# qcc4cp/qcc

Measured on AMD Instinct MI355X. Metric: gate-applies/sec (2^30-amplitude units), QFT, higher is better.
Workload: dtype f64; 1 GPU; 30-qubit QFT complex128, 465 gates/step (qc.qft order), basis-state input, state resident in HBM, 2^30 amplitudes per GPU [BASELINE config 2]; qubits=30, fusion=1

## Files before the change

### qcc_amd/csrc/planner.h

```cpp
#pragma once
#include <sched.h>
#include <stdint.h>

#include <algorithm>
#include <atomic>
#include <cassert>
#include <cmath>
#include <cstdio>
#include <cstdlib>
#include <cstring>
#include <exception>
#include <new>
#include <string>
#include <thread>
#include <vector>

#include "../../include/qcc_hip.h"

namespace qh {

struct GateRec {
  uint64_t ctl_mask;
  int tgt;
  double g[8];
  uint64_t neg_mask = 0;
  uint8_t ghost = 0, variant = 0;
  uint8_t force_dense = 0;
};

inline bool is_diag(const double g[8]) {
  return g[2] == 0.0 && g[3] == 0.0 && g[4] == 0.0 && g[5] == 0.0;
}
inline bool is_one(double re, double im) { return re == 1.0 && im == 0.0; }
inline bool plan_diag(const double g[8], int tgt) {
  return is_diag(g) && (tgt < 0 || !(g[0] == 0.0 && g[1] == 0.0));
}
inline bool plan_diag(const GateRec &r) { return !r.force_dense && plan_diag(r.g, r.tgt); }

constexpr int kLaneBits = 6;
constexpr int kLaneLow = 3;
constexpr int kLaneHi = 3;
constexpr int kMaxLaneHiBit = 27;
constexpr int kMaxRegBits = 6;
inline int max_reg_bits(int bw) { return bw == 128 ? 5 : 6; }
constexpr int kMaxWaveBits = 2;
constexpr int kMaxSweepOps = 1024;
constexpr int kMaxInsertBits = 12;
constexpr int kMaxSlabBits = 3;

enum : uint32_t { OP_DENSE_REG = 0, OP_DENSE_LANE = 1, OP_DIAG = 2,
                  OP_LSWAP = 3,
                  OP_WSWAP = 4 };
enum : uint32_t { OPF_DEFER_C = 1, OPF_USE_C = 2, OPF_REAL = 4,
                  OPF_BFLY = 8, OPF_BFLY_SHIFT = 4,
                  OPF_LANE_DPP = 128, OPF_SWAP_RI = 256,
                  OPF_GHOST = 1024,
                  OPF_ROT_P = 2048, OPF_ROT_M = 4096 };

inline bool env_flag(const char *name, bool dflt) {
  const char *e = getenv(name);
  return e ? atoi(e) != 0 : dflt;
}

inline int env_int(const char *name, int dflt) {
  const char *e = getenv(name);
  return e ? atoi(e) : dflt;
}

struct PlanSwitches {
  bool wave_pinned = false;
  int wave_bits = 1;
  bool split_lanes = true;
  int max_rb = kMaxRegBits;
  bool bfly = true, propagate_x = true, defer_diag = true, rot_fuse = true;
  int lane_valu = 1, seats = 1;
  bool search = true, search_wb2 = true;
  bool steps_pinned = false; uint64_t steps = 0;
  int streams = 0;
  int only_wb = -1, pick = -1;
  int tiles_wb = 0;
  std::vector<std::vector<int>> tiles;
  bool threads = true, log = false, dag = false, verbose = false;

  static PlanSwitches from_env() {
    PlanSwitches w;
    if (const char *e = getenv("QH_WAVE_BITS")) { w.wave_pinned = true; w.wave_bits = std::max(0, std::min(kMaxWaveBits, atoi(e))); }
    w.split_lanes = env_flag("QH_SPLIT_LANES", true);
    w.max_rb = std::max(2, std::min(kMaxRegBits, env_int("QH_SWEEP_RB", kMaxRegBits)));
    w.bfly = env_flag("QH_BFLY", true), w.propagate_x = env_flag("QH_PROPAGATE_X", true);
    w.defer_diag = env_flag("QH_DEFER_DIAG", true), w.rot_fuse = env_flag("QH_ROT_FUSE", true);
    w.lane_valu = env_int("QH_LANE_VALU", 1), w.seats = env_int("QH_SEATS", 1);
    w.search = env_flag("QH_PLAN_SEARCH", true), w.search_wb2 = env_flag("QH_PLAN_SEARCH_WB2", true);
    if (const char *e = getenv("QH_PLAN_SEARCH_STEPS")) { w.steps_pinned = true; w.steps = strtoull(e, nullptr, 10); }
    if (const char *e = getenv("QH_PLAN_SEARCH_STREAMS")) w.streams = std::max(1, std::min(8, atoi(e)));
// ... 248 lines not shown
      pending.swap(rest);
      ++*nsweeps;
    }
  }

  void canonical_records(const std::vector<GateRec> &pending, std::vector<PassRec> *rec0, int back[64], uint64_t *movable) {
    const uint64_t always = (1ull << lane_low_) - 1;
    int canon[64], ncanon = lane_low_;
    for (int b = 0; b < 64; ++b) canon[b] = b < lane_low_ ? b : -1;
    auto canon_mask = [&](uint64_t m) {
      uint64_t o = 0;
      for (uint64_t t = m; t; t &= t - 1) {
        const int b = __builtin_ctzll(t);
        if (canon[b] < 0) canon[b] = ncanon++;
        o |= 1ull << canon[b];
      }
      return o;
    };
    rec0->resize(pending.size());
    uint64_t dense_used = 0;
    for (size_t i = 0; i < pending.size(); ++i) {
      const GateRec &r = pending[i];
      const bool diag = plan_diag(r);
      const uint64_t tb = canon_mask((r.tgt >= 0) ? (1ull << r.tgt) : 0);
      const uint64_t cb = canon_mask((r.ctl_mask | r.neg_mask) & ((1ull << nloc_) - 1));
      (*rec0)[i] = PassRec{diag ? 0 : tb, cb | (diag ? tb : 0), 1, tb ? __builtin_ctzll(tb) : -1};
      if (!diag) dense_used |= tb;
    }
    for (int b = 0; b < 64; ++b) back[b] = -1;
    for (int b = 0; b < 64; ++b) if (canon[b] >= 0) back[canon[b]] = b;
    *movable = dense_used & ~always;
  }
  static void build_dag(const std::vector<PassRec> &rec0, std::vector<int> *node_bit, std::vector<std::vector<int>> *succ,
                        std::vector<std::vector<int>> *pred) {
    int last_dense[64];
    std::vector<int> need[64];
    for (int b = 0; b < 64; ++b) last_dense[b] = -1;
    for (const PassRec &r : rec0) {
      if (!r.dense_bits) {
        for (uint64_t t = r.diag_bits; t; t &= t - 1) {
          const int b = __builtin_ctzll(t);
          for (uint64_t u = r.diag_bits & ~(1ull << b); u; u &= u - 1)
            if (last_dense[__builtin_ctzll(u)] >= 0) need[b].push_back(last_dense[__builtin_ctzll(u)]);
        }
        continue;
      }
      const int v = (int)node_bit->size(), tb = r.tgt;
      node_bit->push_back(tb);
      succ->emplace_back();
      pred->emplace_back();
      std::vector<int> ps;
      if (last_dense[tb] >= 0) ps.push_back(last_dense[tb]);
      for (int u : need[tb]) ps.push_back(u);
      for (uint64_t t = r.diag_bits; t; t &= t - 1) if (last_dense[__builtin_ctzll(t)] >= 0) ps.push_back(last_dense[__builtin_ctzll(t)]);
      std::sort(ps.begin(), ps.end());
      ps.erase(std::unique(ps.begin(), ps.end()), ps.end());
      for (int u : ps) { (*succ)[u].push_back(v); (*pred)[v].push_back(u); }
      need[tb].clear();
      last_dense[tb] = v;
      for (uint64_t t = r.diag_bits; t; t &= t - 1) need[__builtin_ctzll(t)].push_back(v);
    }
  }
  std::string dag_json(const std::vector<GateRec> &queue) {
    std::vector<GateRec> pending;
    std::vector<uint64_t> alg;
    uint64_t noops = 0;
    prepare(queue, &pending, &alg, &noops);
    std::vector<PassRec> rec0;
    int back[64];
    uint64_t movable = 0;
    canonical_records(pending, &rec0, back, &movable);
    std::vector<int> node_bit;
    std::vector<std::vector<int>> succ, pred;
    build_dag(rec0, &node_bit, &succ, &pred);
    std::string o = "{\"line_bits\":" + std::to_string(lane_low_) + ",\"cap_per_wave_bits\":[" + std::to_string(lane_hi_ + rb_cap_) + "," +
                    std::to_string(lane_hi_ + rb_cap_ + 1) + "," + std::to_string(lane_hi_ + rb_cap_ + 2) + "],\"target_bit\":[";
    for (size_t g = 0; g < node_bit.size(); ++g) o += (g ? "," : "") + std::to_string(back[node_bit[g]]);
    o += "],\"edges\":[";
    bool first = true;
    for (size_t u = 0; u < succ.size(); ++u)
      for (int v : succ[u]) { o += (first ? "[" : ",[") + std::to_string(u) + "," + std::to_string(v) + "]"; first = false; }
    return o + "]}";
  }
  bool search_levels(const std::vector<GateRec> &queue, size_t K, uint64_t change_budget, uint64_t stream,
                     std::vector<std::vector<int>> *tiles_out, uint64_t *changes_used = nullptr) {
    if (changes_used) *changes_used = 0;
    if (K < 2 || K > 8) return false;
    std::vector<GateRec> pending;
    std::vector<uint64_t> alg;
    uint64_t noops = 0;
    prepare(queue, &pending, &alg, &noops);
    std::vector<PassRec> rec0;
    int back[64];
    uint64_t movable = 0;
    canonical_records(pending, &rec0, back, &movable);
    const uint64_t always = (1ull << lane_low_) - 1;
    const int cap = lane_hi_ + rb_cap_ + max_wave_;
    if ((size_t)popc(movable) > K * (size_t)cap) return false;
    std::vector<int> node_bit;
    std::vector<std::vector<int>> succ, pred;
    build_dag(rec0, &node_bit, &succ, &pred);
    const int ng = (int)node_bit.size();
    if (!ng) return false;
    std::vector<int> depth(ng, 0);
    int maxd = 0;
    for (int u = 0; u < ng; ++u) for (int v : succ[u]) { depth[v] = std::max(depth[v], depth[u] + 1); maxd = std::max(maxd, depth[v]); }
    std::vector<int> chain[64];
    for (int g = 0; g < ng; ++g) chain[node_bit[g]].push_back(g);
    std::vector<int8_t> L(ng);
    int occ[64][8], ntile[8];
    uint64_t changes = 0;
    auto set_level = [&](int g, int to) {
      const int q = node_bit[g], from = L[g];
      ++changes;
      if (!((always >> q) & 1)) {
        if (--occ[q][from] == 0) --ntile[from];
        if (occ[q][to]++ == 0) ++ntile[to];
      }
      L[g] = (int8_t)to;
    };
    auto init = [&]() {
      memset(occ, 0, sizeof occ);
      memset(ntile, 0, sizeof ntile);
      for (int g = 0; g < ng; ++g) {
        L[g] = (int8_t)std::min<int>((int)K - 1, depth[g] * (int)K / (maxd + 1));
        const int q = node_bit[g];
        if (!((always >> q) & 1) && occ[q][L[g]]++ == 0) ++ntile[L[g]];
      }
    };
    auto cost = [&](int *over) {
      long sq = 0;
      int o = 0;
      for (size_t s = 0; s < K; ++s) { sq += (long)ntile[s] * ntile[s]; if (ntile[s] > cap) o += ntile[s] - cap; }
      *over = o;
      return (long)o * 100000 + sq;
    };
    std::vector<int> stk;
    std::vector<std::pair<int, int8_t>> undo;
    auto move = [&](int g, bool down) {
      const int to = L[g] + (down ? -1 : 1);
      if (to < 0 || to >= (int)K) return false;
      stk.assign(1, g);
      undo.emplace_back(g, L[g]);
      set_level(g, to);
      while (!stk.empty()) {
        const int u = stk.back();
        stk.pop_back();
        for (int v : down ? pred[u] : succ[u])
          if (down ? L[v] > to : L[v] < to) { undo.emplace_back(v, L[v]); set_level(v, to); stk.push_back(v); }
      }
      return true;
    };
    auto revert = [&]() { for (size_t i = undo.size(); i-- > 0;) set_level(undo[i].first, undo[i].second); undo.clear(); };
    uint64_t rng = 0x9e3779b97f4a7c15ull * (2 * stream + 1);
    auto rnd = [&](uint32_t n) { rng ^= rng << 13; rng ^= rng >> 7; rng ^= rng << 17; return (uint32_t)((rng >> 11) % n); };
    constexpr long kRestart = 1500;
    constexpr int kTenure = 7;
    std::vector<long> tabu((size_t)ng * 2);
    std::vector<int> cands;
    bool found = false;
    for (long walk = 0; !found; ++walk) {
      init();
      std::fill(tabu.begin(), tabu.end(), -1);
      int over = 0, best_over = 0;
      long best_key = cost(&best_over);
      over = best_over;
      for (long it = 0; it < kRestart && over > 0; ++it) {
        if (++changes > change_budget) goto out;
        if (walk == 0 && it == 400 && best_over > 4) goto out;
        cands.clear();
        for (size_t s = 0; s < K; ++s) {
          if (ntile[s] <= cap) continue;
          for (uint64_t t = movable; t; t &= t - 1) {
            const int q = __builtin_ctzll(t);
            if (!occ[q][s]) continue;
            int first = -1, last = -1;
            for (int g : chain[q]) if (L[g] == (int8_t)s) { if (first < 0) first = g; last = g; }
            cands.push_back(first * 2);
            cands.push_back(last * 2 + 1);
          }
        }
        long bk = 1L << 60;
        int bm = -1, ties = 0;
        for (int m : cands) {
          undo.clear();
          if (!move(m >> 1, m & 1)) continue;
          int o = 0;
          const long k = cost(&o);
          revert();
          if (tabu[m] > it && !(o < best_over)) continue;
          if (k < bk) { bk = k; bm = m; ties = 1; }
          else if (k == bk && rnd((uint32_t)++ties) == 0) bm = m;
        }
        if (bm < 0) continue;
        undo.clear();
        move(bm >> 1, bm & 1);
        const long k = cost(&over);
        for (const auto &u : undo) tabu[(size_t)u.first * 2 + ((bm & 1) ? 0 : 1)] = it + kTenure + (long)rnd(kTenure);
        if (k < best_key) { best_key = k; best_over = over; }
      }
      found = over == 0;
    }
  out:
    if (changes_used) *changes_used = changes;
    if (!found) return false;
    tiles_out->clear();
    for (size_t s = 0; s < K; ++s) {
      std::vector<int> b;
      for (uint64_t t = movable; t; t &= t - 1) if (occ[__builtin_ctzll(t)][s]) b.push_back(back[__builtin_ctzll(t)]);
      std::sort(b.begin(), b.end());
      tiles_out->push_back(b);
    }
    return true;
  }
  void set_tiles(const std::vector<std::vector<int>> &t) { tiles_ = t; }

  PlanResult plan(const std::vector<GateRec> &queue) {
    PlanResult out;
    std::vector<GateRec> pending;
    std::vector<uint64_t> alg;
    prepare(queue, &pending, &alg, &out.noop_gates);
    const uint64_t lm = (1ull << nloc_) - 1;
    std::vector<int> first_tile;
    keep_line_bits_ = !tiles_.empty();
    while (!pending.empty()) {
      std::vector<GateRec> rest;
      std::vector<uint64_t> rest_alg;
      std::vector<uint32_t> rest_w;
      std::vector<int> forced;
      const std::vector<int> *fs = nullptr;
      if (out.sweeps.size() < tiles_.size()) {
        for (int b : tiles_[out.sweeps.size()])
          if (b >= lane_low_ && b < nloc_) forced.push_back(out.final_pos[b]);
        fs = &forced;
      }
      out.sweeps.push_back(build_sweep(pending, alg, &rest, &rest_alg, &rest_w, fs));
      if (out.sweeps.size() == 1) {
        const SweepPlan &f = out.sweeps[0];
        for (int k = 0; k < f.nlanehi(); ++k) first_tile.push_back(f.lanehi[k]);
        for (int k = 0; k < f.rb; ++k) first_tile.push_back(f.regpos[k]);
        for (int k = 0; k < f.nwave; ++k) first_tile.push_back(f.wavepos[k]);
      }
      if (out.sweeps.back().relayout) {
        std::vector<int> ahead;
        if (!rest.empty() && out.sweeps.size() < tiles_.size()) {
          for (int b : tiles_[out.sweeps.size()])
            if (b >= lane_low_ && b < nloc_) ahead.push_back(out.final_pos[b]);
        } else if (!rest.empty()) {
          select_tile_bits(rest, &ahead);
        } else if (out.sweeps.size() > 1) {
          for (int p : first_tile) ahead.push_back(out.final_pos[p]);
        }
        std::sort(ahead.begin(), ahead.end());
        finish_relayout(&out.sweeps.back(), ahead);
        if (unit_segments(out.sweeps.back(), nloc_, nullptr, nullptr) > kMaxUnitSegs)
          finish_relayout(&out.sweeps.back(), std::vector<int>());
      }
      const SweepPlan &done = out.sweeps.back();
      if (done.relayout) {
        auto map_mask = [&](uint64_t m) {
          uint64_t o = m >> nloc_ << nloc_;
          for (uint64_t t = m & lm; t; t &= t - 1) o |= 1ull << done.dest_pos[__builtin_ctzll(t)];
          return o;
        };
        for (GateRec &r : rest) {
          r.ctl_mask = map_mask(r.ctl_mask);
          r.neg_mask = map_mask(r.neg_mask);
          if (r.tgt >= 0 && r.tgt < nloc_) r.tgt = done.dest_pos[r.tgt];
        }
        for (int p = 0; p < nloc_; ++p) out.final_pos[p] = done.dest_pos[out.final_pos[p]];
        out.moved = true;
      }
      pending.swap(rest);
      alg.swap(rest_alg);
      weight_.swap(rest_w);
    }
    return out;
  }

 private:
  int nloc_;
  uint64_t shard_;
  uint64_t amp_bytes_;
  int rb_cap_;
  int lane_low_ = kLaneLow, lane_hi_ = kLaneHi;
  bool split_lanes_;
  bool relayout_;
  bool keep_ghosts_;
  bool butterflies_;
  static constexpr size_t dense_weight_ = 1;
  int max_wave_;
  bool propagate_x_;
  static constexpr bool store_swapped_ = true, lanes_by_count_ = true, lanes_high_ = true, bitfac_ = true, fold_sink_ = true;
  static constexpr int min_table_terms_ = 2;
  bool fold_pending_ = false;
  bool keep_line_bits_ = false;
  double fold_re_ = 1, fold_im_ = 0;
// ... 1076 lines not shown
        const int i = __builtin_ctz(g.reg_mask & ~(1u << best_j));
        for (int t = 0; t < no; ++t) if (others[t] == i) slot = t;
      }
      if (slot < 0) { kept.push_back(g); continue; }
      cmul_acc(&w[2 * slot], &w[2 * slot + 1], g.re, g.im);
      if ((int)k < base_abs) base--;
    }
    if (base < 0) {
      DGroup g{};
      g.reg_mask = 1u << best_j;
      g.re = 1; g.im = 0;
      kept.push_back(g);
      base = (int)kept.size() - 1;
    } else {
      base -= (int)first;
    }
    kept[base].flags |= DG_BITFAC;
    kept[base].tab_off[3] = (uint32_t)(sp->tables.size() / 2);
    for (double x : w) sp->tables.push_back(x);
    sp->groups.resize(first);
    for (const DGroup &g : kept) sp->groups.push_back(g);
  }
};

inline bool plan_has_far_tile(const PlanResult &pr) {
  for (const SweepPlan &sp : pr.sweeps) {
    int far = 0;
    for (int k = 0; k < sp.nlanehi(); ++k) far += sp.lanehi[k] >= 25;
    for (int k = 0; k < sp.rb; ++k) far += sp.regpos[k] >= 25;
    if (far >= 8) return true;
  }
  return false;
}

inline double sweep_op_energy_nj(const SweepPlan &sp) {
  const double nr = (double)(1u << sp.rb);
  double e = 0;
  for (const SweepOp &op : sp.ops) {
    const uint32_t f = op.flags;
    if (f & OPF_GHOST) continue;
    switch (op.kind) {
      case OP_DENSE_REG:
        if ((f & OPF_BFLY) && (f & (OPF_ROT_P | OPF_ROT_M))) e += 3 * nr * 1.58;
        else if (f & OPF_BFLY) e += 2 * nr * 1.5;
        else if (f & OPF_REAL) e += 5 * nr * 1.9;
        else e += (10 * nr + 10) * 1.95;
        break;
      case OP_DENSE_LANE:
        if ((f & OPF_LANE_DPP) && (f & OPF_BFLY)) e += (nr * (op.tb == 2 ? 10 : 6) + 14) * 1.0;
        else if (f & OPF_LANE_DPP) e += (nr * (op.tb == 2 ? 12 : 8) + 20) * 1.1;
        else if (f & OPF_BFLY) e += (2 * nr + 8) * 1.5 + 4 * nr * 1.0;
        else e += (((f & OPF_REAL) ? 4 : 10) * nr + 30) * 1.9 + 4 * nr * 1.0;
        break;
      case OP_LSWAP: e += (2 * nr + 8) * 1.2; break;
      case OP_WSWAP: e += 5 * 1.0 + 2 * nr * 1.0; break;
      case OP_DIAG: {
        bool c_touched = false, c_sign = false;
        for (uint32_t gi = 0; gi < op.n_groups; ++gi) {
          const DGroup &g = sp.groups[op.group_off + gi];
          const double slots = nr / (double)(1u << popc((uint64_t)g.reg_mask));
          const bool general = (g.flags & DG_LTAB) || g.ntab || g.n_oterms;
          const bool sign = g.re == -1.0 && g.im == 0.0 && !(g.flags & DG_LTAB) && !g.ntab;
          if (g.flags & DG_BITFAC) { e += (124 + ((g.lane_mask || general) ? 11 : 0)) * 1.95; continue; }
          if (sign) {
            if (!g.reg_mask) { e += 6 * 1.0; c_touched = c_sign = true; }
            else e += (4 + 2 * slots) * 1.0;
            continue;
          }
          double pro = 0;
          if (general) pro = 4 + 4 * g.ntab + 4 * g.n_oterms + ((g.flags & DG_LTAB) ? 4 : 7);
          else if (g.lane_mask) pro = 11;
          if (!g.reg_mask) { e += (pro + 4) * 1.9; c_touched = true; c_sign = false; }
          else e += 4 * slots * 1.95 + pro * 1.0;
        }
        if (c_touched && !(f & OPF_DEFER_C)) e += (c_sign ? (2 * nr + 1) : 4 * nr) * 1.95;
        break;
      }
      default: break;
    }
  }
  return e;
}

inline double plan_predicted_ms(const PlanResult &pr, int nloc, int bw) {
  double ms = 0;
  for (const SweepPlan &sp : pr.sweeps) {
    const double scale = (double)sp.swept_bytes / (2.0 * 16.0 * (double)(1ull << 30));
    const double e_ops_j = sweep_op_energy_nj(sp) * (double)sp.ntiles * 1e-9;
    const double floor_ms = (sp.nwave >= 2 ? 6.0 : 5.5) * scale;
    ms += std::max(floor_ms, 3.0 * scale + 0.99 * e_ops_j) + (sp.nwave >= 2 ? 0.3 * scale : 0.0);
  }
  (void)nloc; (void)bw;
  return ms;
}

inline unsigned usable_cpus() {
  unsigned n = std::thread::hardware_concurrency();
  cpu_set_t set;
  if (sched_getaffinity(0, sizeof set, &set) == 0) { const int c = CPU_COUNT(&set); if (c > 0 && (!n || (unsigned)c < n)) n = (unsigned)c; }
  for (const char *path : {"/sys/fs/cgroup/cpu.max", "/sys/fs/cgroup/cpu/cpu.cfs_quota_us"}) {
    FILE *f = fopen(path, "r");
    if (!f) continue;
    long long quota = -1, period = 100000;
    char word[32] = {0};
    if (fscanf(f, "%31s %lld", word, &period) >= 1 && strcmp(word, "max") != 0) quota = atoll(word);
    fclose(f);
    if (strstr(path, "cfs_quota")) {
      period = 100000;
      if (FILE *g = fopen("/sys/fs/cgroup/cpu/cpu.cfs_period_us", "r")) { if (fscanf(g, "%lld", &period) != 1) period = 100000; fclose(g); }
    }
    if (quota > 0 && period > 0) { const unsigned q = (unsigned)std::max<long long>(1, quota / period); if (!n || q < n) n = q; }
    break;
  }
  return n;
}

inline PlanResult plan_best(const std::vector<GateRec> &queue, const PlanRequest &rq) {
  const PlanSwitches &sw = rq.sw;
  const int nloc = rq.nloc, bw = rq.bw;
  const bool keep_ghosts = rq.keep_ghosts;
  if (sw.wave_pinned) return Planner(rq).plan(queue);
  if (!sw.tiles.empty()) {
    Planner forced(rq, sw.tiles_wb);
    forced.set_tiles(sw.tiles);
    return forced.plan(queue);
  }
  int best_wb = 1;
  size_t best_n = 0, n_of[kMaxWaveBits + 1] = {0, 0, 0};
  bool have = false, best_far = false, far_of[kMaxWaveBits + 1] = {false, false, false};
  const int only_wb = sw.only_wb;
  for (int wb : {1, 2, 0}) {
    if (only_wb >= 0 && wb != only_wb) continue;
    size_t n = 0;
    bool far = false;
    Planner(rq, wb).skeleton(queue, &n, &far);
    n_of[wb] = n;
    far_of[wb] = far;
    if (!have || (best_far && !far) || (best_far == far && n < best_n)) {
      best_wb = wb;
      best_n = n;
      best_far = far;
      have = true;
    }
    if (best_n <= 1 && !best_far) break;
  }
  Planner chosen(rq, best_wb);
  uint64_t dense_bits = 0;
  for (const GateRec &q : queue) if (q.tgt >= 0 && q.tgt < nloc && !plan_diag(q.g, q.tgt)) dense_bits |= 1ull << q.tgt;
  const int lane_low = bw == 128 ? 3 : 4;
  const int cap0 = (kLaneBits - lane_low) + std::min({sw.max_rb, max_reg_bits(bw), nloc - kLaneBits});
  if (best_n >= 3 && sw.search) {
    const double sweep_us = 2.0 * (double)(bw == 128 ? 16 : 8) * (double)(1ull << nloc) / 5.5e6;
    const uint64_t budget = sw.steps_pinned ? sw.steps : std::min<uint64_t>((uint64_t)(sweep_us * 640.0), 5000000);
    struct Task {
      int wb;
      size_t K;
      uint64_t stream, used = 0;
      bool ok = false, planned = false;
      double ms = 0;
      PlanResult pr;
      std::exception_ptr failed;
    };
    std::vector<Task> tasks;
    const size_t nmovable = (size_t)popc(dense_bits >> lane_low);
    std::vector<std::pair<int, size_t>> shapes;
    for (int wb : {1, 2, 0}) {
      if (budget < 5000) break;
      if (wb != best_wb && (wb == 0 || far_of[wb] || n_of[wb] == 0 || best_n < 4 || (wb == 2 && !sw.search_wb2))) continue;
      if (only_wb >= 0 && wb != only_wb) continue;
      const size_t cap = (size_t)(cap0 + wb), greedy = n_of[wb];
      const size_t kmin = std::max<size_t>({2, (nmovable + cap - 1) / cap, greedy > 3 ? greedy - 3 : 0});
      for (size_t K = kmin; K + 1 <= greedy && K <= best_n && K <= 8; ++K) shapes.emplace_back(wb, K);
    }
    int streams = 6;
    if (const unsigned hw = usable_cpus(); hw && !keep_ghosts && !shapes.empty())
      streams = std::max(1, std::min(6, (int)(hw / shapes.size())));
    if (sw.streams) streams = sw.streams;
    for (const auto &sh : shapes)
      for (int s = 0; s < streams; ++s) { tasks.emplace_back(); tasks.back().wb = sh.first; tasks.back().K = sh.second; tasks.back().stream = (uint64_t)(s + 1); }
    auto run = [&](Task &t) {
      const size_t i = (size_t)(&t - &tasks[0]);
      try {
        std::vector<std::vector<int>> tiles;
        t.ok = Planner(rq, t.wb).search_levels(queue, t.K, budget, t.stream, &tiles, &t.used);
        if (!t.ok) return;
        Planner forced(rq, t.wb);
        forced.set_tiles(tiles);
        t.pr = forced.plan(queue);
        t.planned = t.pr.sweeps.size() <= t.K && !plan_has_far_tile(t.pr);
      } catch (...) { t.failed = std::current_exception(); return; }
      if (t.planned) t.ms = keep_ghosts ? 1000.0 * (double)t.pr.sweeps.size() + 1e-3 * (double)(i + 1) : plan_predicted_ms(t.pr, nloc, bw);
    };
    std::atomic<size_t> next{0};
    auto drain = [&] { for (size_t i; (i = next++) < tasks.size(); ) run(tasks[i]); };
    std::vector<std::thread> pool;
    const size_t workers = sw.threads ? std::min<size_t>(tasks.size(), usable_cpus()) : 0;
    try { while (pool.size() < workers) pool.emplace_back(drain); } catch (...) {}
    PlanResult greedy_plan;
    std::exception_ptr greedy_failed;
    try { greedy_plan = chosen.plan(queue); } catch (...) { greedy_failed = std::current_exception(); next = tasks.size(); }
    drain();
    for (std::thread &x : pool) x.join();
    if (greedy_failed) std::rethrow_exception(greedy_failed);
    const Task *win = nullptr;
    double best_ms = keep_ghosts ? 1000.0 * (double)greedy_plan.sweeps.size() : plan_predicted_ms(greedy_plan, nloc, bw);
    for (const Task &t : tasks)
      if (t.planned && t.pr.sweeps.size() <= greedy_plan.sweeps.size() && t.ms < best_ms) { win = &t; best_ms = t.ms; }
    if (sw.pick >= 0) {
      if ((size_t)sw.pick < tasks.size() && tasks[sw.pick].planned) win = &tasks[sw.pick];
    }
    if (sw.log) {
      for (const Task &t : tasks)
        fprintf(stderr, "[qh plan search]   task %d: wave bits %d K=%zu stream %llu: %s after %llu label changes%s\n", (int)(&t - &tasks[0]), t.wb, t.K, (unsigned long long)t.stream,
                t.failed ? "FAILED (exception)" : t.ok ? "found" : "not found", (unsigned long long)t.used,
                t.planned ? (", " + std::to_string(t.pr.sweeps.size()) + " sweeps, predicted " + std::to_string(t.ms) + " ms").c_str() : "");
      fprintf(stderr, "[qh plan search] greedy: %d wave bit(s), %zu sweeps, predicted %.2f ms; chosen: %s (%zu tasks, budget %llu label changes each)\n", best_wb,
              greedy_plan.sweeps.size(), plan_predicted_ms(greedy_plan, nloc, bw),
              win ? (std::to_string(win->pr.sweeps.size()) + " sweeps with " + std::to_string(win->wb) + " wave bit(s), predicted " + std::to_string(win->ms) + " ms").c_str() : "greedy",
              tasks.size(), (unsigned long long)budget);
    }
    if (keep_ghosts)
      for (const Task &t : tasks) if (t.failed) std::rethrow_exception(t.failed);
    if (win) return win->pr;
    return greedy_plan;
  }
  return chosen.plan(queue);
}

template <class F> int guard_planning(std::string *err, F &&f) {
  try { f(); } catch (const std::bad_alloc &) { *err = "planning: out of host memory"; return QH_ERR_NOMEM; }
  catch (const std::exception &e) { *err = std::string("planning: ") + e.what(); return QH_ERR_ARG; }
  return QH_OK;
}

inline std::string plan_to_json(const std::vector<GateRec> &queue, const PlanRequest &rq) {
  if (rq.nloc < kLaneBits + 2) return "{\"sweeps\":[],\"note\":\"state too small for sweeps\"}";
  PlanResult pr = plan_best(queue, rq);
  std::string s = "{\"noop_gates\":" + std::to_string(pr.noop_gates);
  if (rq.sw.dag)
    s += ",\"dag\":" + Planner(rq, 1).dag_json(queue);
  s += ",\"sweeps\":[";
  char buf[384];
  for (size_t i = 0; i < pr.sweeps.size(); ++i) {
    const SweepPlan &sp = pr.sweeps[i];
    int nd = 0, ndiag = 0, nbf = 0;
    int nswap = 0, ndpp = 0;
    for (auto &o : sp.ops) {
      if (o.kind == OP_LSWAP || o.kind == OP_WSWAP) { nswap++; continue; }
      (o.kind == OP_DIAG ? ndiag : nd)++;
      if (o.flags & OPF_BFLY) nbf++;
      if (o.flags & OPF_LANE_DPP) ndpp++;
    }
    std::string rp = "[";
    for (int k = 0; k < sp.rb; ++k) rp += (k ? "," : "") + std::to_string(sp.regpos[k]);
    rp += "],\"lanehi\":[";
    for (int k = 0; k < sp.nlanehi(); ++k) rp += (k ? "," : "") + std::to_string(sp.lanehi[k]);
    rp += "],\"wavepos\":[";
    for (int k = 0; k < sp.nwave; ++k) rp += (k ? "," : "") + std::to_string(sp.wavepos[k]);
    rp += "]";
    rp += sp.relayout ? ",\"relayout\":1" : ",\"relayout\":0";
    snprintf(buf, sizeof buf,
             "%s{\"gates\":%llu,\"dense_ops\":%d,\"butterfly_ops\":%d,\"dpp_ops\":%d,\"lswap_ops\":%d,\"diag_ops\":%d,\"groups\":%zu,\"oterms\":%zu,\"table_entries\":%zu,"
             "\"regpos\":%s,\"fixed_ones\":%llu,\"ntiles\":%llu,\"alg_bytes\":%llu,\"swept_bytes\":%llu}",
             i ? "," : "", (unsigned long long)sp.gates, nd, nbf, ndpp, nswap, ndiag, sp.groups.size(), sp.oterms.size(),
             sp.tables.size() / 2, rp.c_str(), (unsigned long long)sp.fixed_ones, (unsigned long long)sp.ntiles,
             (unsigned long long)sp.alg_bytes, (unsigned long long)sp.swept_bytes);
    s += buf;
    if (rq.sw.verbose) {
      s.pop_back();
      s += ",\"ops\":[";
      for (size_t k = 0; k < sp.ops.size(); ++k) {
        const SweepOp &o = sp.ops[k];
        snprintf(buf, sizeof buf, "%s{\"kind\":%u,\"tb\":%u,\"flags\":%u,\"cm_reg\":%u,\"cm_thread\":%llu,\"groups\":[",
                 k ? "," : "", o.kind, o.tb, o.flags, o.cm_reg, (unsigned long long)o.cm_thread);
        s += buf;
        for (uint32_t gi = 0; o.kind == OP_DIAG && gi < o.n_groups; ++gi) {
          const DGroup &g = sp.groups[o.group_off + gi];
          snprintf(buf, sizeof buf, "%s[%u,%u,%u,%u,%u,%.17g,%.17g]", gi ? "," : "", g.lane_mask, g.reg_mask, g.flags, g.ntab, g.n_oterms, g.re, g.im);
          s += buf;
        }
        s += "]}";
      }
      s += "]}";
    }
  }
  s += "]}";
  return s;
}

}
```

Before: 27540 gate-applies/s.

## Run plan search in budgeted rounds with pruning and a DAG lower bound

The tabu level search becomes a resumable LevelSearch object, and plan_best runs it over several rounds with doubling budgets. After each round it drops tasks that cannot beat the incumbent plan, and it adds extra streams for promising shapes onto spare CPUs. A new DAG-span lower bound (min_tile_slots) raises the minimum sweep count K so hopeless shapes are never searched. The aim is to cut planning time and spend search effort where it can help, but pruning may drop a search that would have found a better plan, which changes the kernel schedule chosen.

```diff
diff --git a/qcc_amd/csrc/planner.h b/qcc_amd/csrc/planner.h
--- a/qcc_amd/csrc/planner.h
+++ b/qcc_amd/csrc/planner.h
@@ -10,6 +10,8 @@
 #include <cstdlib>
 #include <cstring>
 #include <exception>
+#include <functional>
+#include <memory>
 #include <new>
 #include <string>
 #include <thread>
@@ -424,10 +426,7 @@
       for (int v : succ[u]) { o += (first ? "[" : ",[") + std::to_string(u) + "," + std::to_string(v) + "]"; first = false; }
     return o + "]}";
   }
-  bool search_levels(const std::vector<GateRec> &queue, size_t K, uint64_t change_budget, uint64_t stream,
-                     std::vector<std::vector<int>> *tiles_out, uint64_t *changes_used = nullptr) {
-    if (changes_used) *changes_used = 0;
-    if (K < 2 || K > 8) return false;
+  size_t min_tile_slots(const std::vector<GateRec> &queue, int cap) {
     std::vector<GateRec> pending;
     std::vector<uint64_t> alg;
     uint64_t noops = 0;
@@ -436,125 +435,209 @@
     int back[64];
     uint64_t movable = 0;
     canonical_records(pending, &rec0, back, &movable);
-    const uint64_t always = (1ull << lane_low_) - 1;
-    const int cap = lane_hi_ + rb_cap_ + max_wave_;
-    if ((size_t)popc(movable) > K * (size_t)cap) return false;
     std::vector<int> node_bit;
     std::vector<std::vector<int>> succ, pred;
     build_dag(rec0, &node_bit, &succ, &pred);
-    const int ng = (int)node_bit.size();
-    if (!ng) return false;
-    std::vector<int> depth(ng, 0);
-    int maxd = 0;
-    for (int u = 0; u < ng; ++u) for (int v : succ[u]) { depth[v] = std::max(depth[v], depth[u] + 1); maxd = std::max(maxd, depth[v]); }
-    std::vector<int> chain[64];
-    for (int g = 0; g < ng; ++g) chain[node_bit[g]].push_back(g);
-    std::vector<int8_t> L(ng);
-    int occ[64][8], ntile[8];
-    uint64_t changes = 0;
-    auto set_level = [&](int g, int to) {
-      const int q = node_bit[g], from = L[g];
-      ++changes;
-      if (!((always >> q) & 1)) {
-        if (--occ[q][from] == 0) --ntile[from];
-        if (occ[q][to]++ == 0) ++ntile[to];
-      }
-      L[g] = (int8_t)to;
-    };
-    auto init = [&]() {
-      memset(occ, 0, sizeof occ);
-      memset(ntile, 0, sizeof ntile);
-      for (int g = 0; g < ng; ++g) {
-        L[g] = (int8_t)std::min<int>((int)K - 1, depth[g] * (int)K / (maxd + 1));
-        const int q = node_bit[g];
-        if (!((always >> q) & 1) && occ[q][L[g]]++ == 0) ++ntile[L[g]];
-      }
-    };
-    auto cost = [&](int *over) {
+    const size_t ng = node_bit.size(), nw = (ng + 63) / 64;
+    auto is_movable = [&](int g) { return (movable >> node_bit[g]) & 1; };
+    std::vector<uint64_t> below(ng * nw, 0), above(ng * nw, 0);
+    for (size_t u = ng; u-- > 0;) {
+      below[u * nw + u / 64] |= 1ull << (u % 64);
+      for (int v : succ[u]) for (size_t w = 0; w < nw; ++w) below[u * nw + w] |= below[(size_t)v * nw + w];
+    }
+    for (size_t v = 0; v < ng; ++v) {
+      above[v * nw + v / 64] |= 1ull << (v % 64);
+      for (int u : pred[v]) for (size_t w = 0; w < nw; ++w) above[v * nw + w] |= above[(size_t)u * nw + w];
+    }
+    size_t events = 0;
+    int last[64];
+    for (int b = 0; b < 64; ++b) last[b] = -1;
+    struct Pair { int q; std::vector<uint64_t> span; bool open; };
+    std::vector<Pair> pairs;
+    for (size_t g = 0; g < ng; ++g) {
+      if (!is_movable((int)g)) continue;
+      ++events;
+      const int q = node_bit[g], f = last[q];
+      last[q] = (int)g;
+      if (f < 0) continue;
+      Pair p{q, std::vector<uint64_t>(nw), true};
+      uint64_t targets = 0;
+      for (size_t w = 0; w < nw; ++w) {
+        p.span[w] = below[(size_t)f * nw + w] & above[g * nw + w];
+        for (uint64_t t = p.span[w]; t; t &= t - 1) targets |= 1ull << node_bit[w * 64 + __builtin_ctzll(t)];
+      }
+      if (popc(targets & movable) <= cap) pairs.push_back(std::move(p));
+    }
+    size_t merges = 0, left = pairs.size();
+    std::vector<size_t> in_spans(ng);
+    while (left) {
+      std::fill(in_spans.begin(), in_spans.end(), 0);
+      for (const Pair &p : pairs)
+        if (p.open) for (size_t w = 0; w < nw; ++w) for (uint64_t t = p.span[w]; t; t &= t - 1) ++in_spans[w * 64 + __builtin_ctzll(t)];
+      const size_t x = (size_t)(std::max_element(in_spans.begin(), in_spans.end()) - in_spans.begin());
+      size_t per_qubit[64] = {0};
+      for (Pair &p : pairs)
+        if (p.open && ((p.span[x / 64] >> (x % 64)) & 1)) { ++per_qubit[p.q]; p.open = false; --left; }
+      std::sort(per_qubit, per_qubit + 64, std::greater<size_t>());
+      for (int k = 0; k < cap && k < 64; ++k) merges += per_qubit[k];
+    }
+    return events - merges;
+  }
+
+  class LevelSearch {
+   public:
+    enum State { kRunning, kFound, kGaveUp };
+    LevelSearch(const PlanRequest &rq, int wave_bits, const std::vector<GateRec> &queue, size_t K, uint64_t stream)
+        : K_(K), rng_(0x9e3779b97f4a7c15ull * (2 * stream + 1)) {
+      if (K < 2 || K > 8) { state_ = kGaveUp; return; }
+      Planner pl(rq, wave_bits);
+      std::vector<GateRec> pending;
+      std::vector<uint64_t> alg;
+      uint64_t noops = 0;
+      pl.prepare(queue, &pending, &alg, &noops);
+      std::vector<PassRec> rec0;
+      pl.canonical_records(pending, &rec0, back_, &movable_);
+      always_ = (1ull << pl.lane_low_) - 1;
+      cap_ = pl.lane_hi_ + pl.rb_cap_ + pl.max_wave_;
+      if ((size_t)popc(movable_) > K * (size_t)cap_) { state_ = kGaveUp; return; }
+      build_dag(rec0, &node_bit_, &succ_, &pred_);
+      ng_ = (int)node_bit_.size();
+      if (!ng_) { state_ = kGaveUp; return; }
+      depth_.assign(ng_, 0);
+      for (int u = 0; u < ng_; ++u) for (int v : succ_[u]) { depth_[v] = std::max(depth_[v], depth_[u] + 1); maxd_ = std::max(maxd_, depth_[v]); }
+      for (int g = 0; g < ng_; ++g) chain_[node_bit_[g]].push_back(g);
+      L_.resize(ng_);
+      tabu_.resize((size_t)ng_ * 2);
+    }
+    State state() const { return state_; }
+    uint64_t changes() const { return changes_; }
+    int least_overflow() const { return least_over_; }
+
+    State run(uint64_t change_budget) {
+      constexpr long kRestart = 1500;
+      constexpr int kTenure = 7;
+      while (state_ == kRunning) {
+        if (!in_walk_) {
+          init();
+          std::fill(tabu_.begin(), tabu_.end(), -1);
+          best_key_ = cost(&best_over_);
+          over_ = best_over_;
+          least_over_ = std::min(least_over_, best_over_);
+          it_ = 0;
+          in_walk_ = true;
+        }
+        for (; it_ < kRestart && over_ > 0; ++it_) {
+          if (changes_ + 1 > change_budget) return state_;
+          ++changes_;
+          if (walk_ == 0 && it_ == 400 && best_over_ > kFarOverflow) return state_ = kGaveUp;
+          cands_.clear();
+          for (size_t s = 0; s < K_; ++s) {
+            if (ntile_[s] <= cap_) continue;
+            for (uint64_t t = movable_; t; t &= t - 1) {
+              const int q = __builtin_ctzll(t);
+              if (!occ_[q][s]) continue;
+              int first = -1, last = -1;
+              for (int g : chain_[q]) if (L_[g] == (int8_t)s) { if (first < 0) first = g; last = g; }
+              cands_.push_back(first * 2);
+              cands_.push_back(last * 2 + 1);
+            }
+          }
+          long bk = 1L << 60;
+          int bm = -1, ties = 0;
+          for (int m : cands_) {
+            undo_.clear();
+            if (!move(m >> 1, m & 1)) continue;
+            int o = 0;
+            const long k = cost(&o);
+            revert();
+            if (tabu_[m] > it_ && !(o < best_over_)) continue;
+            if (k < bk) { bk = k; bm = m; ties = 1; }
+            else if (k == bk && rnd((uint32_t)++ties) == 0) bm = m;
+          }
+          if (bm < 0) continue;
+          undo_.clear();
+          move(bm >> 1, bm & 1);
+          const long k = cost(&over_);
+          for (const auto &u : undo_) tabu_[(size_t)u.first * 2 + ((bm & 1) ? 0 : 1)] = it_ + kTenure + (long)rnd(kTenure);
+          if (k < best_key_) { best_key_ = k; best_over_ = over_; }
+          least_over_ = std::min(least_over_, over_);
+        }
+        in_walk_ = false;
+        ++walk_;
+        if (over_ == 0) state_ = kFound;
+      }
+      return state_;
+    }
+    std::vector<std::vector<int>> tiles() const {
+      std::vector<std::vector<int>> out;
+      for (size_t s = 0; s < K_; ++s) {
+        std::vector<int> b;
+        for (uint64_t t = movable_; t; t &= t - 1) if (occ_[__builtin_ctzll(t)][s]) b.push_back(back_[__builtin_ctzll(t)]);
+        std::sort(b.begin(), b.end());
+        out.push_back(b);
+      }
+      return out;
+    }
+    static constexpr int kFarOverflow = 4;
+
+   private:
+    void set_level(int g, int to) {
+      const int q = node_bit_[g], from = L_[g];
+      ++changes_;
+      if (!((always_ >> q) & 1)) {
+        if (--occ_[q][from] == 0) --ntile_[from];
+        if (occ_[q][to]++ == 0) ++ntile_[to];
+      }
+      L_[g] = (int8_t)to;
+    }
+    void init() {
+      memset(occ_, 0, sizeof occ_);
+      memset(ntile_, 0, sizeof ntile_);
+      for (int g = 0; g < ng_; ++g) {
+        L_[g] = (int8_t)std::min<int>((int)K_ - 1, depth_[g] * (int)K_ / (maxd_ + 1));
+        const int q = node_bit_[g];
+        if (!((always_ >> q) & 1) && occ_[q][L_[g]]++ == 0) ++ntile_[L_[g]];
+      }
+    }
+    long cost(int *over) const {
       long sq = 0;
       int o = 0;
-      for (size_t s = 0; s < K; ++s) { sq += (long)ntile[s] * ntile[s]; if (ntile[s] > cap) o += ntile[s] - cap; }
+      for (size_t s = 0; s < K_; ++s) { sq += (long)ntile_[s] * ntile_[s]; if (ntile_[s] > cap_) o += ntile_[s] - cap_; }
       *over = o;
       return (long)o * 100000 + sq;
-    };
-    std::vector<int> stk;
-    std::vector<std::pair<int, int8_t>> undo;
-    auto move = [&](int g, bool down) {
-      const int to = L[g] + (down ? -1 : 1);
-      if (to < 0 || to >= (int)K) return false;
-      stk.assign(1, g);
-      undo.emplace_back(g, L[g]);
+    }
+    bool move(int g, bool down) {
+      const int to = L_[g] + (down ? -1 : 1);
+      if (to < 0 || to >= (int)K_) return false;
+      stk_.assign(1, g);
+      undo_.emplace_back(g, L_[g]);
       set_level(g, to);
-      while (!stk.empty()) {
-        const int u = stk.back();
-        stk.pop_back();
-        for (int v : down ? pred[u] : succ[u])
-          if (down ? L[v] > to : L[v] < to) { undo.emplace_back(v, L[v]); set_level(v, to); stk.push_back(v); }
+      while (!stk_.empty()) {
+        const int u = stk_.back();
+        stk_.pop_back();
+        for (int v : down ? pred_[u] : succ_[u])
+          if (down ? L_[v] > to : L_[v] < to) { undo_.emplace_back(v, L_[v]); set_level(v, to); stk_.push_back(v); }
       }
       return true;
-    };
-    auto revert = [&]() { for (size_t i = undo.size(); i-- > 0;) set_level(undo[i].first, undo[i].second); undo.clear(); };
-    uint64_t rng = 0x9e3779b97f4a7c15ull * (2 * stream + 1);
-    auto rnd = [&](uint32_t n) { rng ^= rng << 13; rng ^= rng >> 7; rng ^= rng << 17; return (uint32_t)((rng >> 11) % n); };
-    constexpr long kRestart = 1500;
-    constexpr int kTenure = 7;
-    std::vector<long> tabu((size_t)ng * 2);
-    std::vector<int> cands;
-    bool found = false;
-    for (long walk = 0; !found; ++walk) {
-      init();
-      std::fill(tabu.begin(), tabu.end(), -1);
-      int over = 0, best_over = 0;
-      long best_key = cost(&best_over);
-      over = best_over;
-      for (long it = 0; it < kRestart && over > 0; ++it) {
-        if (++changes > change_budget) goto out;
-        if (walk == 0 && it == 400 && best_over > 4) goto out;
-        cands.clear();
-        for (size_t s = 0; s < K; ++s) {
-          if (ntile[s] <= cap) continue;
-          for (uint64_t t = movable; t; t &= t - 1) {
-            const int q = __builtin_ctzll(t);
-            if (!occ[q][s]) continue;
-            int first = -1, last = -1;
-            for (int g : chain[q]) if (L[g] == (int8_t)s) { if (first < 0) first = g; last = g; }
-            cands.push_back(first * 2);
-            cands.push_back(last * 2 + 1);
-          }
-        }
-        long bk = 1L << 60;
-        int bm = -1, ties = 0;
-        for (int m : cands) {
-          undo.clear();
-          if (!move(m >> 1, m & 1)) continue;
-          int o = 0;
-          const long k = cost(&o);
-          revert();
-          if (tabu[m] > it && !(o < best_over)) continue;
-          if (k < bk) { bk = k; bm = m; ties = 1; }
-          else if (k == bk && rnd((uint32_t)++ties) == 0) bm = m;
-        }
-        if (bm < 0) continue;
-        undo.clear();
-        move(bm >> 1, bm & 1);
-        const long k = cost(&over);
-        for (const auto &u : undo) tabu[(size_t)u.first * 2 + ((bm & 1) ? 0 : 1)] = it + kTenure + (long)rnd(kTenure);
-        if (k < best_key) { best_key = k; best_over = over; }
-      }
-      found = over == 0;
-    }
-  out:
-    if (changes_used) *changes_used = changes;
-    if (!found) return false;
-    tiles_out->clear();
-    for (size_t s = 0; s < K; ++s) {
-      std::vector<int> b;
-      for (uint64_t t = movable; t; t &= t - 1) if (occ[__builtin_ctzll(t)][s]) b.push_back(back[__builtin_ctzll(t)]);
-      std::sort(b.begin(), b.end());
-      tiles_out->push_back(b);
-    }
-    return true;
-  }
+    }
+    void revert() { for (size_t i = undo_.size(); i-- > 0;) set_level(undo_[i].first, undo_[i].second); undo_.clear(); }
+    uint32_t rnd(uint32_t n) { rng_ ^= rng_ << 13; rng_ ^= rng_ >> 7; rng_ ^= rng_ << 17; return (uint32_t)((rng_ >> 11) % n); }
+
+    size_t K_;
+    uint64_t rng_, always_ = 0, movable_ = 0, changes_ = 0;
+    int cap_ = 0, ng_ = 0, maxd_ = 0, back_[64];
+    std::vector<int> node_bit_, depth_, chain_[64];
+    std::vector<std::vector<int>> succ_, pred_;
+    State state_ = kRunning;
+    std::vector<int8_t> L_;
+    int occ_[64][8], ntile_[8];
+    std::vector<long> tabu_;
+    std::vector<int> stk_, cands_;
+    std::vector<std::pair<int, int8_t>> undo_;
+    long walk_ = 0, it_ = 0, best_key_ = 0;
+    int over_ = 0, best_over_ = 0, least_over_ = 1 << 30;
+    bool in_walk_ = false;
+  };
   void set_tiles(const std::vector<std::vector<int>> &t) { tiles_ = t; }
 
   PlanResult plan(const std::vector<GateRec> &queue) {
@@ -1797,13 +1880,14 @@
   return e;
 }
 
-inline double plan_predicted_ms(const PlanResult &pr, int nloc, int bw) {
+inline double plan_predicted_ms(const PlanResult &pr, int nloc, int bw, int max_wave = kMaxWaveBits) {
   double ms = 0;
   for (const SweepPlan &sp : pr.sweeps) {
+    const int nwave = std::min(sp.nwave, max_wave);
     const double scale = (double)sp.swept_bytes / (2.0 * 16.0 * (double)(1ull << 30));
     const double e_ops_j = sweep_op_energy_nj(sp) * (double)sp.ntiles * 1e-9;
-    const double floor_ms = (sp.nwave >= 2 ? 6.0 : 5.5) * scale;
-    ms += std::max(floor_ms, 3.0 * scale + 0.99 * e_ops_j) + (sp.nwave >= 2 ? 0.3 * scale : 0.0);
+    const double floor_ms = (nwave >= 2 ? 6.0 : 5.5) * scale;
+    ms += std::max(floor_ms, 3.0 * scale + 0.99 * e_ops_j) + (nwave >= 2 ? 0.3 * scale : 0.0);
   }
   (void)nloc; (void)bw;
   return ms;
@@ -1829,6 +1913,8 @@
   }
   return n;
 }
+
+constexpr int kSearchRounds = 5;
 
 inline PlanResult plan_best(const std::vector<GateRec> &queue, const PlanRequest &rq) {
   const PlanSwitches &sw = rq.sw;
@@ -1871,10 +1957,15 @@
       int wb;
       size_t K;
       uint64_t stream, used = 0;
-      bool ok = false, planned = false;
+      enum End { kRunning, kFound, kGaveUp, kDropped, kFailed } end = kRunning;
+      int round = 0;
+      int from_round = 1;
+      uint64_t behind = 0;
+      bool planned = false;
       double ms = 0;
       PlanResult pr;
       std::exception_ptr failed;
+      std::unique_ptr<Planner::LevelSearch> search;
     };
     std::vector<Task> tasks;
     const size_t nmovable = (size_t)popc(dense_bits >> lane_low);
@@ -1884,7 +1975,12 @@
       if (wb != best_wb && (wb == 0 || far_of[wb] || n_of[wb] == 0 || best_n < 4 || (wb == 2 && !sw.search_wb2))) continue;
       if (only_wb >= 0 && wb != only_wb) continue;
       const size_t cap = (size_t)(cap0 + wb), greedy = n_of[wb];
-      const size_t kmin = std::max<size_t>({2, (nmovable + cap - 1) / cap, greedy > 3 ? greedy - 3 : 0});
+      size_t kmin = std::max<size_t>({2, (nmovable + cap - 1) / cap, greedy > 3 ? greedy - 3 : 0});
+      if (kmin + 1 <= greedy && kmin <= best_n && kmin <= 8) {
+        const size_t slots = Planner(rq, wb).min_tile_slots(queue, (int)cap);
+        kmin = std::max(kmin, (slots + cap - 1) / cap);
+        if (sw.log) fprintf(stderr, "[qh plan search] wave bits %d: at least %zu tile slots at %zu per sweep, no tiling below K=%zu (greedy: %zu sweeps)\n", wb, slots, cap, (slots + cap - 1) / cap, greedy);
+      }
       for (size_t K = kmin; K + 1 <= greedy && K <= best_n && K <= 8; ++K) shapes.emplace_back(wb, K);
     }
     int streams = 6;
@@ -1893,46 +1989,119 @@
     if (sw.streams) streams = sw.streams;
     for (const auto &sh : shapes)
       for (int s = 0; s < streams; ++s) { tasks.emplace_back(); tasks.back().wb = sh.first; tasks.back().K = sh.second; tasks.back().stream = (uint64_t)(s + 1); }
-    auto run = [&](Task &t) {
-      const size_t i = (size_t)(&t - &tasks[0]);
+    auto run = [&](size_t i, int round, uint64_t round_budget) {
+      Task &t = tasks[i];
       try {
-        std::vector<std::vector<int>> tiles;
-        t.ok = Planner(rq, t.wb).search_levels(queue, t.K, budget, t.stream, &tiles, &t.used);
-        if (!t.ok) return;
-        Planner forced(rq, t.wb);
-        forced.set_tiles(tiles);
-        t.pr = forced.plan(queue);
-        t.planned = t.pr.sweeps.size() <= t.K && !plan_has_far_tile(t.pr);
-      } catch (...) { t.failed = std::current_exception(); return; }
+        if (!t.search) t.search.reset(new Planner::LevelSearch(rq, t.wb, queue, t.K, t.stream));
+        const Planner::LevelSearch::State st = t.search->run(round_budget - t.behind);
+        t.used = t.search->changes();
+        if (st == Planner::LevelSearch::kRunning) return;
+        t.round = round;
+        t.end = st == Planner::LevelSearch::kFound ? Task::kFound : Task::kGaveUp;
+        if (t.end == Task::kFound) {
+          Planner forced(rq, t.wb);
+          forced.set_tiles(t.search->tiles());
+          t.pr = forced.plan(queue);
+          t.planned = t.pr.sweeps.size() <= t.K && !plan_has_far_tile(t.pr);
+        }
+        t.search.reset();
+      } catch (...) { t.failed = std::current_exception(); t.end = Task::kFailed; t.round = round; t.planned = false; t.search.reset(); return; }
       if (t.planned) t.ms = keep_ghosts ? 1000.0 * (double)t.pr.sweeps.size() + 1e-3 * (double)(i + 1) : plan_predicted_ms(t.pr, nloc, bw);
     };
-    std::atomic<size_t> next{0};
-    auto drain = [&] { for (size_t i; (i = next++) < tasks.size(); ) run(tasks[i]); };
-    std::vector<std::thread> pool;
-    const size_t workers = sw.threads ? std::min<size_t>(tasks.size(), usable_cpus()) : 0;
-    try { while (pool.size() < workers) pool.emplace_back(drain); } catch (...) {}
     PlanResult greedy_plan;
     std::exception_ptr greedy_failed;
-    try { greedy_plan = chosen.plan(queue); } catch (...) { greedy_failed = std::current_exception(); next = tasks.size(); }
-    drain();
-    for (std::thread &x : pool) x.join();
-    if (greedy_failed) std::rethrow_exception(greedy_failed);
-    const Task *win = nullptr;
-    double best_ms = keep_ghosts ? 1000.0 * (double)greedy_plan.sweeps.size() : plan_predicted_ms(greedy_plan, nloc, bw);
-    for (const Task &t : tasks)
-      if (t.planned && t.pr.sweeps.size() <= greedy_plan.sweeps.size() && t.ms < best_ms) { win = &t; best_ms = t.ms; }
+    double greedy_ms = 0;
+    auto incumbent = [&]() -> const Task * {
+      const Task *win = nullptr;
+      double best_ms = greedy_ms;
+      for (const Task &t : tasks)
+        if (t.planned && t.pr.sweeps.size() <= greedy_plan.sweeps.size() && t.ms < best_ms) { win = &t; best_ms = t.ms; }
+      return win;
+    };
+    const double margin_ms = 0.5 * ((double)(bw == 128 ? 16 : 8) * (double)(1ull << nloc)) / (16.0 * (double)(1ull << 30));
+    std::vector<size_t> alive(tasks.size());
+    for (size_t i = 0; i < alive.size(); ++i) alive[i] = i;
+    if (alive.empty()) return chosen.plan(queue);
+    for (int round = 1; round <= kSearchRounds && !alive.empty(); ++round) {
+      const uint64_t round_budget = budget >> (kSearchRounds - round);
+      std::atomic<size_t> next{0};
+      auto drain = [&] { for (size_t k; (k = next++) < alive.size(); ) run(alive[k], round, round_budget); };
+      std::vector<std::thread> pool;
+      const size_t workers = sw.threads ? std::min<size_t>(alive.size() - (round > 1), usable_cpus()) : 0;
+      try { while (pool.size() < workers) pool.emplace_back(drain); } catch (...) {}
+      if (round == 1) {
+        try {
+          greedy_plan = chosen.plan(queue);
+          greedy_ms = keep_ghosts ? 1000.0 * (double)greedy_plan.sweeps.size() : plan_predicted_ms(greedy_plan, nloc, bw);
+        } catch (...) { greedy_failed = std::current_exception(); next = alive.size(); }
+      }
+      drain();
+      for (std::thread &x : pool) x.join();
+      if (greedy_failed) std::rethrow_exception(greedy_failed);
+      const Task *inc = incumbent();
+      const PlanResult &inc_pr = inc ? inc->pr : greedy_plan;
+      const double inc_ms = inc ? inc->ms : greedy_ms;
+      std::vector<size_t> rest;
+      for (size_t i : alive) {
+        Task &t = tasks[i];
+        if (t.end != Task::kRunning) continue;
+        bool drop = false;
+        if (sw.pick < 0) {
+          if (t.K > inc_pr.sweeps.size()) drop = true;
+          else if (t.K == inc_pr.sweeps.size())
+            drop = keep_ghosts ? !(inc && i < (size_t)(inc - &tasks[0])) : !(plan_predicted_ms(inc_pr, nloc, bw, t.wb) < inc_ms - margin_ms);
+        }
+        if (drop) { t.end = Task::kDropped; t.round = round; t.search.reset(); continue; }
+        if (sw.pick < 0 && t.K == inc_pr.sweeps.size() && t.search->least_overflow() > kSearchRounds - (round - t.from_round + 1)) {
+          t.end = Task::kGaveUp; t.round = round; t.search.reset(); continue;
+        }
+        rest.push_back(i);
+      }
+      for (size_t &i : rest) {
+        Task &t = tasks[i];
+        bool led = t.from_round == 1;
+        for (size_t j : rest) led = led || (tasks[j].from_round == 1 && tasks[j].wb == t.wb && tasks[j].K == t.K);
+        if (!led) { t.end = Task::kDropped; t.round = round; t.search.reset(); i = (size_t)-1; }
+      }
+      rest.erase(std::remove(rest.begin(), rest.end(), (size_t)-1), rest.end());
+      alive.swap(rest);
+      if (!sw.streams && !keep_ghosts && round < kSearchRounds) {
+        size_t room = std::max<size_t>(usable_cpus(), alive.size()) - alive.size();
+        std::vector<std::pair<int, size_t>> open;
+        const size_t inc_sweeps = inc_pr.sweeps.size();
+        for (size_t i : alive)
+          if (tasks[i].K < inc_sweeps && tasks[i].search && tasks[i].search->least_overflow() <= Planner::LevelSearch::kFarOverflow &&
+              std::find(open.begin(), open.end(), std::make_pair(tasks[i].wb, tasks[i].K)) == open.end()) open.emplace_back(tasks[i].wb, tasks[i].K);
+        for (bool added = true; room && added; ) {
+          added = false;
+          for (const auto &sh : open) {
+            uint64_t last = 0;
+            for (const Task &t : tasks) if (t.wb == sh.first && t.K == sh.second) last = std::max(last, t.stream);
+            if (!room || last >= 6) continue;
+            tasks.emplace_back();
+            Task &t = tasks.back();
+            t.wb = sh.first, t.K = sh.second, t.stream = last + 1, t.from_round = round + 1, t.behind = round_budget;
+            alive.push_back(tasks.size() - 1);
+            --room, added = true;
+          }
+        }
+      }
+    }
+    const Task *win = incumbent();
     if (sw.pick >= 0) {
       if ((size_t)sw.pick < tasks.size() && tasks[sw.pick].planned) win = &tasks[sw.pick];
     }
     if (sw.log) {
+      static const char *const ends[] = {"not found", "found", "gave up", "dropped", "FAILED (exception)"};
       for (const Task &t : tasks)
-        fprintf(stderr, "[qh plan search]   task %d: wave bits %d K=%zu stream %llu: %s after %llu label changes%s\n", (int)(&t - &tasks[0]), t.wb, t.K, (unsigned long long)t.stream,
-                t.failed ? "FAILED (exception)" : t.ok ? "found" : "not found", (unsigned long long)t.used,
-                t.planned ? (", " + std::to_string(t.pr.sweeps.size()) + " sweeps, predicted " + std::to_string(t.ms) + " ms").c_str() : "");
-      fprintf(stderr, "[qh plan search] greedy: %d wave bit(s), %zu sweeps, predicted %.2f ms; chosen: %s (%zu tasks, budget %llu label changes each)\n", best_wb,
+        fprintf(stderr, "[qh plan search]   task %d: wave bits %d K=%zu stream %llu: %s in round %d after %llu label changes%s\n", (int)(&t - &tasks[0]), t.wb, t.K,
+                (unsigned long long)t.stream, ends[t.end], t.end == Task::kRunning ? kSearchRounds : t.round, (unsigned long long)t.used,
+                ((t.from_round > 1 ? ", started in round " + std::to_string(t.from_round) : std::string()) +
+                 (t.planned ? ", " + std::to_string(t.pr.sweeps.size()) + " sweeps, predicted " + std::to_string(t.ms) + " ms" : std::string())).c_str());
+      fprintf(stderr, "[qh plan search] greedy: %d wave bit(s), %zu sweeps, predicted %.2f ms; chosen: %s (%zu tasks, budget %llu label changes each in %d rounds)\n", best_wb,
               greedy_plan.sweeps.size(), plan_predicted_ms(greedy_plan, nloc, bw),
               win ? (std::to_string(win->pr.sweeps.size()) + " sweeps with " + std::to_string(win->wb) + " wave bit(s), predicted " + std::to_string(win->ms) + " ms").c_str() : "greedy",
-              tasks.size(), (unsigned long long)budget);
+              tasks.size(), (unsigned long long)budget, kSearchRounds);
     }
     if (keep_ghosts)
       for (const Task &t : tasks) if (t.failed) std::rethrow_exception(t.failed);
```

Result: no change. 27570 gate-applies/s (median of 6 runs) (+0.1%).
